# mandt-lab/shallow-ntc

Measured on AMD Instinct MI355X. Metric: decode Mpixels/s + (bpp, PSNR) on Kodak, two_layer_syn, higher is better.
Workload: dtype f32

## Files before the change

### shallow-ntc_amd/csrc/bf3_gemm.hip

```cpp
#include <algorithm>
#include <type_traits>
#include "sntc_internal.h"

namespace sntc {

typedef float f32x4 __attribute__((ext_vector_type(4)));
typedef float f32x16 __attribute__((ext_vector_type(16)));
typedef unsigned u32x4 __attribute__((ext_vector_type(4)));
typedef __bf16 bf16x8 __attribute__((ext_vector_type(8)));

namespace {

constexpr unsigned kOOR = 0x80000000u;
constexpr int kSpin = 1 << 22;

__device__ __forceinline__ float act_of(float v, int act) {
  switch (act) {
    case SNTC_ACT_RELU: return fmaxf(v, 0.0f);
    case SNTC_ACT_LEAKY_RELU: return v >= 0.0f ? v : 0.2f * v;
    case SNTC_ACT_SIGMOID: return 1.0f / (1.0f + expf(-v));
    default: return v;
  }
}

// ... 453 lines not shown
  using I1 = std::integral_constant<int, 1>;

  int mBc = 0, mBn = 0, mBn2 = 0;
  int mPc = 0, mP1 = 0, mP2 = 0;
  int nP = 0, nP_buf = 0, c_last = 0;
  int pm[NS - 1];
  auto start_piece = [&](const Piece& p, int rb) {
    init_loader(p, rb);
    const int n = __builtin_amdgcn_readfirstlane(p.k1 - p.k0);
    if (HALO) {
      issued = 0;
      const int c0 = ld_cc;
      c_last = __builtin_amdgcn_readfirstlane((p.k1 - 1) / g_T);
      rd_t = ld_t; rd_tx = ld_tx; rd_buf = 0;
      rd_shift = h_shift0 + ld_ty * (h_rowjump + (g_tw - 1) * h_coljump) + ld_tx * h_coljump;
      issue_patch(c0, 0);
      mPc = issued;
      if (h_nbufs == 3 && c0 + 1 <= c_last) issue_patch(c0 + 1, 1);
      mP1 = issued;
      mP2 = issued;
      nP = c0 + h_nbufs - 1;
      nP_buf = h_nbufs - 1;
#pragma unroll
      for (int q = 0; q < NS - 1; ++q) {
        if (q < n) issue(q);
        pm[q] = issued;
      }
      mBc = pm[0];
      mBn = pm[1];
    } else {
      if (n > 0) issue(0);
      if (n > 1) issue(1);
    }
  };

  int rb = 0;
  write_rinfo(P, rb);
  __syncthreads();
  start_piece(P, rb);
  while (true) {
    const int n = __builtin_amdgcn_readfirstlane(P.k1 - P.k0);
    if (P.consume >= 0) {
      if (tid == 0) {
        int spins = 0;
        while (__hip_atomic_load(a.sk_flags + P.consume, __ATOMIC_RELAXED, __HIP_MEMORY_SCOPE_AGENT) == 0) {
          __builtin_amdgcn_s_sleep(8);
          if (++spins > kSpin) {
            __hip_atomic_fetch_or(kargs().status, 1, __ATOMIC_RELAXED, __HIP_MEMORY_SCOPE_AGENT);
            break;
          }
        }
        __builtin_amdgcn_fence(__ATOMIC_ACQUIRE, "agent");
        asm volatile("s_waitcnt vmcnt(0)" ::: "memory");
      }
      __syncthreads();
      const __amdgpu_buffer_rsrc_t sr = __builtin_amdgcn_make_buffer_rsrc(
          a.sk_slab + (size_t)P.consume * (TM * TN * 16 * NT), 0, TM * TN * 16 * NT * 4, 0x00020000);
#pragma unroll
      for (int i = 0; i < TM; ++i)
#pragma unroll
        for (int j = 0; j < TN; ++j)
#pragma unroll
          for (int q = 0; q < 4; ++q) {
            const u32x4 v = __builtin_amdgcn_raw_buffer_load_b128(sr, tid * 16, ((i * TN + j) * 4 + q) * NT * 16, 0);
            const f32x4 f = __builtin_bit_cast(f32x4, v);
            acc[i][j][4 * q] = f[0]; acc[i][j][4 * q + 1] = f[1]; acc[i][j][4 * q + 2] = f[2]; acc[i][j][4 * q + 3] = f[3];
          }
    } else {
#pragma unroll
      for (int i = 0; i < TM; ++i)
#pragma unroll
        for (int j = 0; j < TN; ++j)
#pragma unroll
          for (int e = 0; e < 16; ++e) acc[i][j][e] = 0.0f;
    }

    Frag F;
    int s_cur = 0, s_n1 = 1, s_n2 = 2;
    if constexpr (HALO && DBUF) {
      Frag G;
      wait_vm(issued - max(mBc, mPc));
      __builtin_amdgcn_s_barrier();
      __builtin_amdgcn_sched_barrier(0);
      int mq[NS - 2];
#pragma unroll
      for (int q = 0; q < NS - 2; ++q) mq[q] = pm[q + 1];
      int s_rd = 0, s_is = NS - 1;
      auto mf = [&](const Frag& Fc, bool on, int q) {
        const int t = q / (TM * TN), i = (q / TN) % TM, j2 = q % TN;
        constexpr int PA[6] = {2, 0, 1, 1, 0, 0};
        constexpr int PB[6] = {0, 2, 1, 0, 1, 0};
        if (on && !SNTC_DBG(a, 64))
          acc[i][j2] = __builtin_amdgcn_mfma_f32_32x32x16_bf16(Fc.a[PA[t]][i], Fc.b[PB[t]][j2], acc[i][j2], 0, 0, 0);
        __builtin_amdgcn_sched_barrier(0);
      };
      auto step = [&](auto EDGE_, int j, Frag& Fc, Frag& Fn) {
        constexpr bool EDGE = decltype(EDGE_)::value;
        const bool mm = !EDGE || j >= 0, rd = (!EDGE || j + 1 < n) && (!SNTC_DBG(a, 8) || j < 1);
        static_assert(TM == 2 && TN == 2, "the slices below are laid out for a 64 x 64 wave tile (24 MFMAs per stage)");
        const char* src[TM];
        bool in[TM];
        const char* bsrc = ring + s_rd * SLOT + fb;
        int q = 0;
#pragma unroll
        for (int i = 0; i < TM; ++i) {
          const int prow = r_row[i] + rd_shift;
// ... 288 lines not shown
```

### shallow-ntc_amd/csrc/common.hip

```cpp
#include <algorithm>
#include <cstring>
#include "sntc_internal.h"

namespace sntc {

static thread_local std::string g_last_error;

void set_error(const std::string& msg) { g_last_error = msg; }

int fail(int code, const std::string& msg) {
  g_last_error = msg;
  return code;
}

int hip_fail(hipError_t e, const char* what) {
  g_last_error = std::string("HIP error in ") + what + ": " + hipGetErrorString(e);
  (void)hipGetLastError();
  return SNTC_ERR_HIP;
}

__global__ void __launch_bounds__(256) zero_words_kernel(uint32_t* __restrict__ p, size_t n) {
  for (size_t i = blockIdx.x * (size_t)blockDim.x + threadIdx.x; i < n; i += (size_t)gridDim.x * blockDim.x) p[i] = 0u;
}

int zero_async(void* p, size_t bytes, hipStream_t stream) {
  if (bytes == 0) return SNTC_OK;
  if ((bytes & 3u) || (reinterpret_cast<uintptr_t>(p) & 3u)) return fail(SNTC_ERR_BAD_SHAPE, "zero_async: unaligned range");
  const size_t n = bytes / 4;
  const int blocks = (int)std::min<size_t>((n + 255) / 256, 1024);
  hipLaunchKernelGGL(zero_words_kernel, dim3(blocks), dim3(256), 0, stream, reinterpret_cast<uint32_t*>(p), n);
  hipError_t e = hipGetLastError();
  if (e != hipSuccess) return hip_fail(e, "zero_async");
  return SNTC_OK;
}

}

extern "C" const char* sntc_last_error(void) { return sntc::g_last_error.c_str(); }

extern "C" int sntc_version(void) { return SNTC_VERSION; }

extern "C" int sntc_device_count(void) {
  int n = 0;
  if (hipGetDeviceCount(&n) != hipSuccess) {
    (void)hipGetLastError();
    return 0;
  }
  return n;
}

extern "C" int sntc_device_arch(int device, char* buf, size_t buflen) {
  if (!buf || buflen == 0) return sntc::fail(SNTC_ERR_BAD_SHAPE, "sntc_device_arch: null buffer");
  hipDeviceProp_t prop;
  if (sntc_device_count() <= device || device < 0) return sntc::fail(SNTC_ERR_NO_DEVICE, "no such HIP device");
  SNTC_HIP(hipGetDeviceProperties(&prop, device));
  std::strncpy(buf, prop.gcnArchName, buflen - 1);
  buf[buflen - 1] = 0;
  return SNTC_OK;
}
```

### shallow-ntc_amd/csrc/conv_plan.hip

```cpp
#include <algorithm>
#include <cstdio>
#include <cstdlib>
#include <array>
#include <atomic>
#include <map>
#include <mutex>
#include <cstdlib>
#include <vector>
#include "sntc_internal.h"

namespace sntc {

struct PackDesc {
  const float* w;
  float* wp;
  const int* taps;
  const unsigned* cols;
  int T, Cin, Cout, K, Ncol, kw, s, pt, pl, phase_mode, slab_major, out_major, bf3, rowpack;
};

__device__ __forceinline__ void pack_element(const PackDesc& d, size_t idx) {
  const int col = (int)(idx / d.K);
  const int k = (int)(idx - (size_t)col * d.K);
  float v = 0.0f;
// ... 102 lines not shown
  } g[kMaxGroups];
  float* bias = nullptr;
  int tile = 0;
  bool bf3 = false;
  bool rowpack = false;
  bool s3 = false;
  bool out_major = false;
  int dma = -1;
  bool no_stream_k = false;
  bool force_stream_k = false;
  int colm = -1;
  bool no_halo = false;
  float* w2f = nullptr;
  struct Choice { int variant = 0; int sk = 0; };
  mutable std::mutex tune_mu;
  std::map<std::array<int, 4>, Choice> tuned;
};
typedef sntc_conv_plan::Choice TuneChoice;

static const GGInstance* base_instance(const sntc_conv_plan* p, int v) {
  return p->s3 ? gg_find(v, kLoadVec, kStageDma, kFormPresplit) : gg_find(v, kLoadVec, kStageRing, kFormPlain);
}

extern "C" int sntc_conv_plan_set_tile(sntc_conv_plan* p, int variant) {
  if (!p) return fail(SNTC_ERR_BAD_SHAPE, "sntc_conv_plan_set_tile: null plan");
  if (variant != 0 && !base_instance(p, variant)) return fail(SNTC_ERR_UNSUPPORTED, "sntc_conv_plan_set_tile: unknown tile variant");
  p->tile = variant;
  return SNTC_OK;
}

static bool plan_dma(const sntc_conv_plan* p) {
  return p->dma > 0 && p->vec && p->d.prologue == SNTC_PRO_NONE && !p->bf3;
}

extern "C" int sntc_conv_plan_set_schedule(sntc_conv_plan* p, int flags) {
  if (!p) return fail(SNTC_ERR_BAD_SHAPE, "sntc_conv_plan_set_schedule: null plan");
  p->no_stream_k = (flags & 1) == 0;
  p->force_stream_k = (flags & 8) != 0;
  p->no_halo = (flags & 16) != 0;
  p->colm = (flags & 32) ? ((flags & 64) ? 1 : 0) : -1;
  p->dma = (flags & 4) ? ((flags & 2) ? 1 : 0) : -1;
  return SNTC_OK;
}

extern "C" void sntc_conv_plan_destroy(sntc_conv_plan* p) {
  if (!p) return;
  for (int i = 0; i < kMaxGroups; ++i) {
    if (p->g[i].wp) (void)hipFree(p->g[i].wp);
    if (p->g[i].taps) (void)hipFree(p->g[i].taps);
    if (p->g[i].cols) (void)hipFree(p->g[i].cols);
  }
  if (p->bias) (void)hipFree(p->bias);
  if (p->w2f) (void)hipFree(p->w2f);
  delete p;
}

static bool fusable_second(const sntc_conv_plan* p) {
  const sntc_conv_desc& b = p->d;
  return !p->up && !p->bf3 && b.kh == 1 && b.kw == 1 && b.stride == 1 && b.cin == 96 && b.cout == 192 &&
         b.prologue == SNTC_PRO_NONE && b.act == SNTC_ACT_NONE && p->ngroups == 1 && p->g[0].K == 96;
}

static int pack_fused_second(sntc_conv_plan* p, hipStream_t stream) {
  if (!fusable_second(p)) return SNTC_OK;
  if (!p->w2f) SNTC_HIP(hipMalloc(&p->w2f, sizeof(float) * 2 * 3 * 12 * 64 * 4));
  hipLaunchKernelGGL(pack_fused_w2_kernel, dim3(72), dim3(256), 0, stream, p->g[0].wp, p->w2f, p->g[0].K, p->g[0].Ncol);
  SNTC_HIP(hipGetLastError());
  return SNTC_OK;
}

static int build_plan(sntc_conv_plan* p, const float* weight, const float* bias, hipStream_t stream) {
  const sntc_conv_desc& d = p->d;
  const int k = d.kh, s = d.stride;
  struct HostGrp { std::vector<int> taps; std::vector<unsigned> cols; int q0y = 0, q0x = 0; bool uniform = true; };
  std::vector<HostGrp> groups;
  auto enc = [](int oyo, int oxo, int ch) { return ((unsigned)(oyo + 128) << 24) | ((unsigned)(oxo + 128) << 16) | (unsigned)ch; };

  if (!p->phase_mode) {
    HostGrp hg;
    for (int ky = 0; ky < d.kh; ++ky)
      for (int kx = 0; kx < (p->rowpack ? 1 : d.kw); ++kx) hg.taps.push_back((ky << 16) | kx);
    for (int ch = 0; ch < d.cout; ++ch) hg.cols.push_back(enc(0, 0, ch));
    groups.push_back(std::move(hg));
  } else {
    auto classes = [&](int kk, std::vector<std::pair<int, std::vector<int>>>& out) {
      for (int phi = 0; phi < s; ++phi) {
        const int cnt = (kk - phi + s - 1) / s;
        if (cnt <= 0) return false;
        bool found = false;
        for (auto& c : out)
          if (c.first == cnt) { c.second.push_back(phi); found = true; }
        if (!found) out.push_back({cnt, {phi}});
      }
      std::sort(out.begin(), out.end(), [](const auto& a, const auto& b) { return a.first > b.first; });
      return true;
    };
    std::vector<std::pair<int, std::vector<int>>> cy, cx;
    if (!classes(d.kh, cy) || !classes(d.kw, cx))
      return fail(SNTC_ERR_UNSUPPORTED, "transposed convolution with kernel < stride is not supported");
    for (auto& a : cy)
      for (auto& b : cx) {
        HostGrp hg;
        for (int jy = 0; jy < a.first; ++jy)
          for (int jx = 0; jx < b.first; ++jx) hg.taps.push_back((jy << 16) | jx);
        for (int py : a.second)
          for (int px : b.second)
// ... 511 lines not shown
  return conv_launch_info(p, n, h, w, 0, variant, nblocks, nullptr);
}

static int conv_forward_impl(const sntc_conv_plan* p, const sntc_conv_plan* p2, const float* x, int n, int h, int w, float* y,
                             const float* res, const float* aux, void* workspace, size_t workspace_bytes, void* stream,
                             const TuneChoice* force = nullptr, int ncols = 0) {
  if (!p || !x || !y) return fail(SNTC_ERR_BAD_SHAPE, "sntc_conv_forward: null argument");
  if (ncols != 0) {
    if (const char* why = columns_error(p, ncols)) return fail(SNTC_ERR_UNSUPPORTED, why);
    if (p2) return fail(SNTC_ERR_UNSUPPORTED, "column-limited launches: not the fused pair");
  }
  if (n < 1) return fail(SNTC_ERR_BAD_SHAPE, "sntc_conv_forward: empty batch");
  const sntc_conv_desc& d = p->d;
  const int epilogue = p2 ? p2->d.epilogue : d.epilogue;
  if (epilogue != SNTC_EPI_STORE && !res) return fail(SNTC_ERR_BAD_SHAPE, "epilogue needs `res`");
  if (epilogue == SNTC_EPI_GATE && !aux) return fail(SNTC_ERR_BAD_SHAPE, "gate epilogue needs `aux`");
  Geo g;
  int rc = geometry(p, h, w, &g);
  if (rc) return rc;
  const int64_t M = (int64_t)n * g.Qh * g.Qw;
  const int64_t x_bytes = (int64_t)n * h * w * d.cin * (p->s3 ? 6 : 4);
  if (M > 0x7fffffffLL || x_bytes >= (1LL << 31))
    return fail(SNTC_ERR_BAD_SHAPE, "sntc_conv_forward: input tensor must be < 2 GiB (32-bit buffer offsets); split the batch");
  if (p2 && M * p2->d.cout >= (1LL << 32)) return fail(SNTC_ERR_BAD_SHAPE, "sntc_conv_forward_fused: output too large; split the batch");
  const Sched sc = force ? schedule(p, g, n, false, force, ncols) : plan_schedule(p, g, n, h, w, p2 != nullptr, ncols);
  if (!sc.inst) return fail(SNTC_ERR_UNSUPPORTED, "sntc_conv_forward: no compiled instance for this plan and tile variant");
  const int64_t ws_floats = workspace_floats(p, M, sc, ncols);
  if (ws_floats > 0 && (!workspace || workspace_bytes < (size_t)ws_floats * 4))
    return fail(SNTC_ERR_BAD_SHAPE, "sntc_conv_forward: this call needs sntc_conv_workspace_bytes() of workspace "
                                    "(split-K slabs / stream-K hand-off)");
  const GGInstance& inst = *sc.inst;
  const Work wk = work_of(p, inst, M, ncols);
  if (sc.sk && wk.units != sc.units) return fail(SNTC_ERR_HIP, "sntc_conv_forward: schedule and launch disagree about the work units");
  GGArgs a{};
  a.ksplit = sc.ksplit;
  a.slab = static_cast<float*>(workspace);
  a.x = x; a.y = y; a.bias = p->bias; a.res = res; a.aux = aux;
  a.x_bytes = (unsigned)x_bytes;
  a.N = n; a.H = h; a.W = w; a.Cin = d.cin;
  a.Qh = g.Qh; a.Qw = g.Qw; a.M = (int)M;
  a.Ho = g.Ho; a.Wo = g.Wo; a.Cout = ncols > 0 ? ncols : d.cout;
  a.sA = g.sA; a.tstep = g.tstep; a.offy = g.offy; a.offx = g.offx; a.sO = g.sO;
  a.act = d.act; a.epi = epilogue; a.pro = d.prologue;
  a.ntm = wk.ntm;
  a.ngroups = p->ngroups;
  if (p2) { a.w2f = p2->w2f; a.bias2 = p2->bias; a.Cout2 = p2->d.cout; }
  a.status = gg_status_word();
  if (!a.status) return fail(SNTC_ERR_HIP, "sntc_conv_forward: the device tables of the current device are not initialised");
  a.sk = sc.sk ? 1 : 0;
  a.nworkers = sc.workers;
  a.units = wk.units;
  if (sc.sk) {
    a.sk_slab = static_cast<float*>(workspace);
    a.sk_flags = reinterpret_cast<int*>(a.sk_slab + (size_t)sc.workers * inst.slab_floats);
    a.slab = nullptr;
    if (int zrc = zero_async(a.sk_flags, sizeof(int) * sc.workers, (hipStream_t)stream)) return zrc;
  }
  int nb = 0;
  size_t slab_off = 0;
  for (int gi = 0; gi < p->ngroups; ++gi) {
    GGGroup& G = a.g[gi];
    G.wp = p->g[gi].wp; G.taps = p->g[gi].taps; G.cols = reinterpret_cast<const int*>(p->g[gi].cols);
    G.T = p->g[gi].T; G.K = p->g[gi].K; G.Ncol = launch_cols(p, gi, ncols); G.tw = p->g[gi].tw;
    G.ntn = wk.ntn[gi];
    G.steps = G.K / kStage;
    G.blk0 = nb;
    G.tile0 = wk.tile0[gi];
    G.unit0 = wk.unit0[gi];
    nb += G.ntn * a.ntm * sc.ksplit;
    G.slab_off = slab_off;
    G.q0y = p->g[gi].q0y; G.q0x = p->g[gi].q0x;
    slab_off += (size_t)sc.ksplit * M * G.Ncol;
  }
  a.tps = wk.tps;
  a.ups = (int)wk.ups;
  if (p->s3) a.order = p->dma == 0 ? 0 : 1;
  rc = gg_launch(inst, a, sc.sk ? sc.workers : nb, (hipStream_t)stream);
  if (rc || sc.sk || sc.ksplit <= 1) return rc;
  return gg_reduce_launch(a, (hipStream_t)stream);
}

extern "C" int sntc_conv_forward(const sntc_conv_plan* p, const float* x, int n, int h, int w, float* y,
                                 const float* res, const float* aux, void* workspace, size_t workspace_bytes,
                                 void* stream) {
  return conv_forward_impl(p, nullptr, x, n, h, w, y, res, aux, workspace, workspace_bytes, stream);
}

static void tune_candidates(const sntc_conv_plan* p, const Geo& g, int n, std::vector<std::pair<TuneChoice, Sched>>* out, int ncols = 0) {
  for (int v = 1; v <= kMaxVariant; ++v) {
    if (!base_instance(p, v)) continue;
    for (int sk = 1; sk >= 0; --sk) {
      TuneChoice c;
      c.variant = v;
      c.sk = sk;
      const Sched s = schedule(p, g, n, false, &c, ncols);
      if (!s.inst || s.inst->variant != v || (sk && !s.sk)) continue;
      out->push_back({c, s});
    }
  }
}

static int64_t conv_tune_workspace_bytes(const sntc_conv_plan* p, int n, int h, int w, int ncols) {
  if (!p) return 0;
  Geo g;
  if (geometry(p, h, w, &g)) return 0;
  std::vector<std::pair<TuneChoice, Sched>> cand;
  tune_candidates(p, g, n, &cand, ncols);
  int64_t m = 0;
  for (auto& c : cand) m = std::max(m, workspace_floats(p, (int64_t)n * g.Qh * g.Qw, c.second, ncols));
// ... 127 lines not shown

extern "C" int sntc_conv_columns_candidates(const sntc_conv_plan* p, int n, int h, int w, int ncols, int* variants, int* stream_k,
                                            int capacity) {
  if (columns_error(p, ncols)) { (void)fail(SNTC_ERR_UNSUPPORTED, columns_error(p, ncols)); return -1; }
  return conv_plan_candidates(p, n, h, w, ncols, variants, stream_k, capacity);
}

extern "C" int sntc_conv_columns_set_choice(sntc_conv_plan* p, int n, int h, int w, int ncols, int variant, int stream_k) {
  if (const char* why = columns_error(p, ncols)) return fail(SNTC_ERR_UNSUPPORTED, why);
  return conv_plan_set_choice(p, n, h, w, ncols, variant, stream_k);
}

extern "C" int sntc_conv_plan_drop_choice(sntc_conv_plan* p, int n, int h, int w, int ncols) {
  if (!p) return fail(SNTC_ERR_BAD_SHAPE, "sntc_conv_plan_drop_choice: null plan");
  std::lock_guard<std::mutex> lk(p->tune_mu);
  p->tuned.erase({n, h, w, ncols});
  return SNTC_OK;
}

extern "C" int sntc_conv_plan_clear_tuning(sntc_conv_plan* p) {
  if (!p) return fail(SNTC_ERR_BAD_SHAPE, "sntc_conv_plan_clear_tuning: null plan");
  std::lock_guard<std::mutex> lk(p->tune_mu);
  p->tuned.clear();
  return SNTC_OK;
}

static const char* fused_pair_error(const sntc_conv_plan* p, const sntc_conv_plan* p2) {
  if (!p || !p2) return "null plan";
  const sntc_conv_desc& a = p->d;
  if (p->up || p2->up || p->bf3 || p2->bf3) return "forward convolutions in fp32 only";
  if (!p->vec || a.cout != 96 || a.stride != 1 || a.prologue != SNTC_PRO_NONE || a.epilogue != SNTC_EPI_STORE || p->ngroups != 1)
    return "first plan: stride-1 convolution with Cin % 16 == 0 and 96 output channels, plain store";
  if (!fusable_second(p2) || !p2->w2f) return "second plan: 1x1 convolution 96 -> 192 without activation";
  return nullptr;
}

extern "C" int sntc_conv_fusable(const sntc_conv_plan* p, const sntc_conv_plan* p2) { return fused_pair_error(p, p2) ? 0 : 1; }

extern "C" int64_t sntc_conv_fused_workspace_bytes(const sntc_conv_plan* p, int n, int h, int w) {
  if (!p) return 0;
  Geo g;
  if (geometry(p, h, w, &g)) return 0;
  return 4 * workspace_floats(p, (int64_t)n * g.Qh * g.Qw, schedule(p, g, n, true));
}

extern "C" int sntc_conv_forward_fused(const sntc_conv_plan* p, const sntc_conv_plan* p2, const float* x, int n, int h, int w, float* y,
                                       const float* res, const float* aux, void* workspace, size_t workspace_bytes,
                                       void* stream) {
  if (const char* why = fused_pair_error(p, p2)) return fail(SNTC_ERR_UNSUPPORTED, why);
  return conv_forward_impl(p, p2, x, n, h, w, y, res, aux, workspace, workspace_bytes, stream);
}

extern "C" int sntc_conv_set_stream_k(int enabled) {
  g_stream_k_enabled.store(enabled ? 1 : 0, std::memory_order_relaxed);
  return SNTC_OK;
}

extern "C" int sntc_conv_get_stream_k(void) { return g_stream_k_enabled.load(std::memory_order_relaxed); }

__global__ void status_exchange_kernel(int* word, int* out) { *out = atomicExch(word, 0); }
__global__ void status_or_kernel(int* word, int flags) { atomicOr(word, flags); }

extern "C" int sntc_conv_status(int* flags, void* stream) {
  if (!flags) return fail(SNTC_ERR_BAD_SHAPE, "sntc_conv_status: null argument");
  int rc = gg_init();
  if (rc) return rc;
  int* word = gg_status_word();
  hipStream_t s = (hipStream_t)stream;
  hipLaunchKernelGGL(status_exchange_kernel, dim3(1), dim3(1), 0, s, word, word + 1);
  SNTC_HIP(hipGetLastError());
  SNTC_HIP(hipMemcpyAsync(flags, word + 1, sizeof(int), hipMemcpyDeviceToHost, s));
  SNTC_HIP(hipStreamSynchronize(s));
  return SNTC_OK;
}

extern "C" int sntc_conv_status_inject(int flags, void* stream) {
  int rc = gg_init();
  if (rc) return rc;
  hipLaunchKernelGGL(status_or_kernel, dim3(1), dim3(1), 0, (hipStream_t)stream, gg_status_word(), flags);
  SNTC_HIP(hipGetLastError());
  return SNTC_OK;
}
```

### shallow-ntc_amd/csrc/gather_gemm_kernel.h

```cpp
#pragma once
#include <algorithm>
#include <cstdlib>
#include <mutex>
#include <type_traits>
#include "sntc_internal.h"

namespace sntc {

typedef float f32x4 __attribute__((ext_vector_type(4)));
typedef float f32x16 __attribute__((ext_vector_type(16)));
typedef unsigned u32x4 __attribute__((ext_vector_type(4)));

constexpr unsigned kOutOfRange = 0x80000000u;
constexpr int kSpinLimit = 1 << 22;

__device__ __forceinline__ float apply_act(float v, int act) {
  switch (act) {
    case SNTC_ACT_RELU: return fmaxf(v, 0.0f);
    case SNTC_ACT_LEAKY_RELU: return v >= 0.0f ? v : 0.2f * v;
    case SNTC_ACT_SIGMOID: return 1.0f / (1.0f + expf(-v));
    default: return v;
  }
}

// ... 525 lines not shown
  f32x16 acc[TM][TN];
  auto mfma3 = [&](const Frag3& F) {
    constexpr int PA[6] = {2, 0, 1, 1, 0, 0};
    constexpr int PB[6] = {0, 2, 1, 0, 1, 0};
#pragma unroll
    for (int t = 0; t < (BF3 ? 6 : 0); ++t)
#pragma unroll
      for (int i = 0; i < TM; ++i)
#pragma unroll
        for (int j = 0; j < TN; ++j)
          acc[i][j] = __builtin_amdgcn_mfma_f32_32x32x16_bf16(F.a[BF3 ? PA[t] : 0][i], F.b[BF3 ? PB[t] : 0][j], acc[i][j], 0, 0, 0);
  };
  auto mfma_group = [&](const Frag& F) {
    if (SNTC_DBG(a, 64)) return;
#pragma unroll
    for (int e = 0; e < 4; ++e)
#pragma unroll
      for (int i = 0; i < TM; ++i)
#pragma unroll
        for (int j = 0; j < TN; ++j)
          acc[i][j] = FUSE2 ? __builtin_amdgcn_mfma_f32_32x32x2f32(F.b[j][e], F.a[i][e], acc[i][j], 0, 0, 0)
                            : __builtin_amdgcn_mfma_f32_32x32x2f32(F.a[i][e], F.b[j][e], acc[i][j], 0, 0, 0);
  };

  int rb = 0;
  Regs R0, R1;
  write_rinfo(P, rb);
  __syncthreads();
  init_loader(P, rb);
  int dma_issued = 0;
  if (DMA) {
    const int n = P.k1 - P.k0;
    for (; dma_issued < RING - 1 && dma_issued < n; ++dma_issued) dma_stage(dma_issued);
  } else {
    const int n = P.k1 - P.k0;
    if (n > 0) load_regs(R0);
    if (RBUF && n > 1) load_regs(R1);
  }

  while (true) {
    const int n = P.k1 - P.k0;
    if (P.consume >= 0) {
      if (tid == 0) {
        int spins = 0;
        while (__hip_atomic_load(a.sk_flags + P.consume, __ATOMIC_RELAXED, __HIP_MEMORY_SCOPE_AGENT) == 0) {
          __builtin_amdgcn_s_sleep(8);
          if (++spins > kSpinLimit) {
            __hip_atomic_fetch_or(fresh_args().status, 1, __ATOMIC_RELAXED, __HIP_MEMORY_SCOPE_AGENT);
            break;
          }
        }
        __builtin_amdgcn_fence(__ATOMIC_ACQUIRE, "agent");
        asm volatile("s_waitcnt vmcnt(0)" ::: "memory");
      }
      __syncthreads();
      const __amdgpu_buffer_rsrc_t sr = __builtin_amdgcn_make_buffer_rsrc(
          a.sk_slab + (size_t)P.consume * (TM * TN * 16 * 256), 0, TM * TN * 16 * 256 * 4, 0x00020000);
#pragma unroll
      for (int i = 0; i < TM; ++i)
#pragma unroll
        for (int j = 0; j < TN; ++j)
#pragma unroll
          for (int q = 0; q < 4; ++q) {
            const f32x4 v = buf_load(sr, (unsigned)tid * 16u, (unsigned)((i * TN + j) * 4 + q) * 4096u);
            acc[i][j][4 * q] = v[0]; acc[i][j][4 * q + 1] = v[1]; acc[i][j][4 * q + 2] = v[2]; acc[i][j][4 * q + 3] = v[3];
          }
    } else {
#pragma unroll
      for (int i = 0; i < TM; ++i)
#pragma unroll
        for (int j = 0; j < TN; ++j)
#pragma unroll
          for (int e = 0; e < 16; ++e) acc[i][j][e] = 0.0f;
    }

    Frag F0, F1;
    if (DMA) {
      for (; dma_issued < RING - 1 && dma_issued < n; ++dma_issued) dma_stage(dma_issued);
      using Yes = std::integral_constant<bool, true>;
      using No = std::integral_constant<bool, false>;
      auto wait_first = [&](auto I) {
        constexpr int i = decltype(I)::value;
        if constexpr (i > 2) {
          if (n >= i) { dma_wait(std::integral_constant<int, i - 2>{}); return true; }
        }
        return false;
      };
      if (!first_of_desc<RING - 1, 3>(wait_first)) dma_wait(std::integral_constant<int, 0>{});
      __builtin_amdgcn_s_barrier();
      __builtin_amdgcn_sched_barrier(0);
      if (n > 0) read_frag(F0, 0, 0);
      auto dstep = [&](int j, auto LD, auto PF, auto REM) {
        if (decltype(LD)::value) dma_stage((j + RING - 1) & (RING - 1));
        read_frag(F1, j & (RING - 1), 1);
        mfma_group(F0);
        if (decltype(PF)::value) read_frag(F0, (j + 1) & (RING - 1), 0);
        mfma_group(F1);
        if (decltype(LD)::value) {
          constexpr int NW = A_CH + B_CH, NR = TM + TN, NM = 4 * TM * TN;
          __builtin_amdgcn_sched_group_barrier(0x008, 1, 0);
          __builtin_amdgcn_sched_group_barrier(0x020, NW, 0);
          __builtin_amdgcn_sched_group_barrier(0x008, 1, 0);
          __builtin_amdgcn_sched_group_barrier(0x100, NR, 0);
          __builtin_amdgcn_sched_group_barrier(0x008, NM - 2, 0);
          __builtin_amdgcn_sched_group_barrier(0x008, 1, 0);
          __builtin_amdgcn_sched_group_barrier(0x100, NR, 0);
// ... 283 lines not shown
```

### shallow-ntc_amd/csrc/sntc_internal.h

```cpp
#pragma once
#include <hip/hip_runtime.h>
#include <stdint.h>
#include <string>
#include "../../include/sntc.h"

namespace sntc {

void set_error(const std::string& msg);
int fail(int code, const std::string& msg);
int hip_fail(hipError_t e, const char* what);
int zero_async(void* p, size_t bytes, hipStream_t stream);

#define SNTC_HIP(expr)                                         \
  do {                                                         \
    hipError_t _e = (expr);                                    \
    if (_e != hipSuccess) return ::sntc::hip_fail(_e, #expr);  \
  } while (0)

constexpr int kMaxGroups = 4;

#ifdef SNTC_DIAG
#define SNTC_DBG(a, bit) (((a).dbg & (bit)) != 0)
#else
#define SNTC_DBG(a, bit) false
#endif

struct GGGroup {
  const float* wp;
  const int* taps;
  const int* cols;
  int T;
  int tw;
  int K;
  int Ncol;
  int ntn;
  int blk0;
  size_t slab_off;
  int q0y, q0x;
  int steps;
  int tile0;
  long long unit0;
};

struct GGArgs {
  const float* x;
  float* y;
  const float* bias;
  const float* res;
  const float* aux;
  unsigned x_bytes;
  int N, H, W, Cin;
  int Qh, Qw, M;
  int Ho, Wo, Cout;
  int sA, tstep, offy, offx, sO;
  int act, epi, pro;
  int ntm;
  int ksplit;
  float* slab;
  int sk;
  int nworkers;
  long long units;
  int tps, ups;
  float* sk_slab;
  int* sk_flags;
// ... 60 lines not shown
```

### shallow-ntc_amd/csrc/syn_fused.hip

```cpp
#include <algorithm>
#include <cmath>
#include <cstdio>
#include <cstdlib>
#include <cstring>
#include <mutex>
#include <vector>
#include "sntc_internal.h"

#include "rb_common.h"

namespace sntc {
namespace syn {

using rb::buf_load;
using rb::buf_store;
using rb::kOOB;

constexpr int kNT = 3;
constexpr int kRows = 32 * kNT;
constexpr int kUnit = kRows * 16;
constexpr int kRing = 8;
constexpr int kLead = 5;
constexpr int kPSlots = 3;
constexpr int kPPMax = 512;
// ... 440 lines not shown
        for (int c = 0; c < CP; ++c) {
          const int vi = sl * CP + c;
          tv[c] = acc[vi >> 4][vi & 15] + bias[c];
        }
        float o[CH];
        if (act == 1 || act == 2) {
          float av[CH];
#pragma unroll
          for (int ic = 0; ic < CH; ++ic) av[ic] = fabsf(tv[ic]);
          f32x2 nrm[CH / 2];
#pragma unroll
          for (int jp = 0; jp < CH / 2; ++jp) nrm[jp] = *reinterpret_cast<const f32x2*>(beta + 2 * jp);
#pragma unroll
          for (int ic = 0; ic < CH; ++ic)
#pragma unroll
            for (int jp = 0; jp < CH / 2; ++jp) {
              const f32x2 g = *reinterpret_cast<const f32x2*>(gamma + ic * CH + 2 * jp);
              const f32x2 pr = g * av[ic];
              nrm[jp] = nrm[jp] + pr;
            }
          if (act == 1) {
#pragma unroll
            for (int jc = 0; jc < CH; ++jc) o[jc] = tv[jc] * nrm[jc >> 1][jc & 1];
          } else {
#pragma unroll
            for (int jc = 0; jc < CH; ++jc) o[jc] = tv[jc] / nrm[jc >> 1][jc & 1];
          }
        } else if (act == 3) {
#pragma unroll
          for (int jc = 0; jc < CH; ++jc) o[jc] = fmaxf(tv[jc], 0.0f);
        } else if (act == 4) {
#pragma unroll
          for (int jc = 0; jc < CH; ++jc) o[jc] = tv[jc] >= 0.0f ? tv[jc] : 0.2f * tv[jc];
        } else {
#pragma unroll
          for (int jc = 0; jc < CH; ++jc) o[jc] = tv[jc];
        }
        if (RES) {
#pragma unroll
          for (int jc = 0; jc < CH; ++jc) o[jc] = o[jc] + tv[CH + jc];
        }
        const unsigned ph0 = up->ph[sl], ph1 = up->ph[SPH + sl];
        const unsigned ph = h ? ph1 : ph0;
        const int ry = (int)(ph >> 8), rx = (int)(ph & 255u);
        const bool ok = pvalid && ph != 0xffffffffu;
        const unsigned off = ok ? (unsigned)(((qy * a.s + ry) * Wo + qx * a.s + rx) * (CH * 4)) : kOOB;
#pragma unroll
        for (int c4 = 0; c4 < CH; c4 += 4) buf_store(vs, f32x4{o[c4], o[c4 + 1], o[c4 + 2], o[c4 + 3]}, off, c4 * 4);
      }
    }
    if (!more) break;
  }
  asm volatile("s_waitcnt vmcnt(0)" ::: "memory");
}

__global__ void __launch_bounds__(256) syn_pack_kernel(const float* __restrict__ w, const SynUnit* __restrict__ units, int nunits,
                                                        SynGeom G, int nslab, int total_steps, float* __restrict__ wpack) {
  const size_t total = (size_t)total_steps * kUnit;
  for (size_t idx = blockIdx.x * (size_t)blockDim.x + threadIdx.x; idx < total; idx += (size_t)gridDim.x * blockDim.x) {
    const int gstep = (int)(idx / kUnit);
    const int rem = (int)(idx - (size_t)gstep * kUnit);
    const int R = rem >> 4, pos = rem & 15;
    const int k16 = (((pos >> 2) ^ ((R >> 2) & 3)) << 2) + (pos & 3);
    int u = 0;
    for (int i = 1; i < nunits; ++i)
      if (gstep >= units[i].step0) u = i;
    const SynUnit U = units[u];
    const int local = gstep - U.step0;
    const int cc = local / U.ns, j = local - cc * U.ns;
    wpack[idx] = pack_value(G, U, cc, j, R, k16, w);
  }
}

__global__ void syn_tables_kernel(const float* b1, const float* beta, const float* gamma, int cp, int ch, float* out) {
  const int i = blockIdx.x * blockDim.x + threadIdx.x;
  if (i < cp) out[i] = b1 ? b1[i] : 0.0f;
  else if (i < cp + ch) out[i] = beta ? beta[i - cp] : 1.0f;
  else if (i < cp + ch + ch * ch) out[i] = gamma ? gamma[i - cp - ch] : 0.0f;
}

struct HostPlan {
  SynGeom G{};
  int ch = 0, has_res = 0;
  std::vector<SynUnit> units;
  int total_steps = 0;
  int nslab = 0;
};

static bool dim_ok(int k, int s, int pt) {
  for (int r = 0; r < s; ++r) {
    const int phi = (r + pt) % s, qo = (r + pt) / s, cnt = (k - phi + s - 1) / s;
    if (cnt < 1 || qo > 1 || qo - cnt + 1 < -1) return false;
  }
  return true;
}

static unsigned phase_mask(const SynGeom& G, int ry, int rx) {
  unsigned m = 0;
  for (int si = 0; si < 9; ++si) {
    const int dy = 1 - si / 3, dx = 1 - si % 3;
    const int phy = (ry + G.pt) % G.s, qoy = (ry + G.pt) / G.s, cy = (G.k - phy + G.s - 1) / G.s;
    const int phx = (rx + G.pt) % G.s, qox = (rx + G.pt) / G.s, cx = (G.k - phx + G.s - 1) / G.s;
    const int jy = qoy - dy, jx = qox - dx;
    if (jy >= 0 && jy < cy && jx >= 0 && jx < cx) m |= 1u << si;
  }
  return m;
// ... 101 lines not shown
  int rc = SNTC_OK;
  int num_cus = 0;
};
SynDevice g_syndev[kMaxDev];

template <int CP, bool RES>
static int set_attr() {
  SNTC_HIP(hipFuncSetAttribute(reinterpret_cast<const void*>(&syn_kernel<CP, RES>), hipFuncAttributeMaxDynamicSharedMemorySize,
                               (int)SynCfg<CP, RES>::LDS));
  return SNTC_OK;
}

static int syn_init(int* num_cus) {
  int dev = 0;
  SNTC_HIP(hipGetDevice(&dev));
  if (dev < 0 || dev >= kMaxDev) return fail(SNTC_ERR_UNSUPPORTED, "device index beyond the synthesis tables");
  SynDevice& D = g_syndev[dev];
  std::call_once(D.once, [&] {
    D.rc = [&]() -> int {
      hipDeviceProp_t prop;
      SNTC_HIP(hipGetDeviceProperties(&prop, dev));
      D.num_cus = prop.multiProcessorCount;
      if (int rc = set_attr<12, false>()) return rc;
      if (int rc = set_attr<24, false>()) return rc;
      if (int rc = set_attr<24, true>()) return rc;
      if (int rc = set_attr<48, false>()) return rc;
      if (int rc = set_attr<48, true>()) return rc;
      return SNTC_OK;
    }();
  });
  *num_cus = D.num_cus;
  return D.rc;
}

}
}

using namespace sntc;
using namespace sntc::syn;

struct sntc_syn_plan {
  HostPlan P;
  int act_kind = 0;
  float* wpack = nullptr;
  SynUnit* units = nullptr;
  float* tables = nullptr;
  int max_workgroups = 0;
};

static void syn_free(sntc_syn_plan* p) {
  if (p->wpack) (void)hipFree(p->wpack);
  if (p->units) (void)hipFree(p->units);
  if (p->tables) (void)hipFree(p->tables);
  delete p;
}

static int syn_pack(sntc_syn_plan* p, const float* w1, const float* b1, const float* beta, const float* gamma, hipStream_t s) {
  const HostPlan& P = p->P;
  const size_t total = (size_t)P.total_steps * kUnit;
  const int blocks = (int)std::min<size_t>((total + 255) / 256, 4096);
  hipLaunchKernelGGL(syn_pack_kernel, dim3(blocks), dim3(256), 0, s, w1, p->units, (int)P.units.size(), P.G, P.nslab, P.total_steps, p->wpack);
  const int nt = P.G.cp + P.ch + P.ch * P.ch;
  hipLaunchKernelGGL(syn_tables_kernel, dim3((nt + 255) / 256), dim3(256), 0, s, b1, beta, gamma, P.G.cp, P.ch, p->tables);
  hipError_t e = hipGetLastError();
  if (e != hipSuccess) return hip_fail(e, "synthesis weight packing");
  return SNTC_OK;
}

extern "C" int sntc_syn_supported(int k, int stride, int cin, int ch, int has_res) {
  HostPlan P;
  if (k < 1 || stride < 1 || ch < 1) return 0;
  return build_host_plan(k, stride, cin, ch, has_res ? 1 : 0, &P) == SNTC_OK ? 1 : 0;
}

extern "C" int sntc_syn_plan_create(int k, int stride, int cin, int ch, int has_res, int act_kind, const float* w1, const float* b1,
                                    const float* beta, const float* gamma, void* stream, sntc_syn_plan** plan) {
  if (!plan || !w1) return fail(SNTC_ERR_BAD_SHAPE, "sntc_syn_plan_create: null argument");
  if (act_kind < 0 || act_kind > 4) return fail(SNTC_ERR_UNSUPPORTED, "sntc_syn_plan_create: unknown activation");
  if ((act_kind == 1 || act_kind == 2) && (!beta || !gamma)) return fail(SNTC_ERR_BAD_SHAPE, "sntc_syn_plan_create: GDN parameters missing");
  if (k < 1 || stride < 1 || ch < 1) return fail(SNTC_ERR_BAD_SHAPE, "sntc_syn_plan_create: bad sizes");
  auto* p = new sntc_syn_plan();
  if (int rc = build_host_plan(k, stride, cin, ch, has_res ? 1 : 0, &p->P)) { delete p; return rc; }
  int cus = 0;
  if (int rc = syn_init(&cus)) { delete p; return rc; }
  p->act_kind = act_kind;
  const HostPlan& P = p->P;
  const int nt = P.G.cp + P.ch + P.ch * P.ch;
  if (hipMalloc(&p->wpack, sizeof(float) * (size_t)P.total_steps * kUnit) != hipSuccess ||
      hipMalloc(&p->units, sizeof(SynUnit) * P.units.size()) != hipSuccess || hipMalloc(&p->tables, sizeof(float) * nt) != hipSuccess) {
    syn_free(p);
    return fail(SNTC_ERR_HIP, "sntc_syn_plan_create: out of device memory");
  }
  hipStream_t s = (hipStream_t)stream;
  if (hipMemcpyAsync(p->units, P.units.data(), sizeof(SynUnit) * P.units.size(), hipMemcpyHostToDevice, s) != hipSuccess ||
      hipStreamSynchronize(s) != hipSuccess) {
    syn_free(p);
    return fail(SNTC_ERR_HIP, "sntc_syn_plan_create: unit table upload");
  }
  if (int rc = syn_pack(p, w1, b1, beta, gamma, s)) { syn_free(p); return rc; }
  *plan = p;
  return SNTC_OK;
}

extern "C" int sntc_syn_plan_update(sntc_syn_plan* p, const float* w1, const float* b1, const float* beta, const float* gamma, void* stream) {
  if (!p || !w1) return fail(SNTC_ERR_BAD_SHAPE, "sntc_syn_plan_update: null argument");
  if ((p->act_kind == 1 || p->act_kind == 2) && (!beta || !gamma)) return fail(SNTC_ERR_BAD_SHAPE, "sntc_syn_plan_update: GDN parameters missing");
  return syn_pack(p, w1, b1, beta, gamma, (hipStream_t)stream);
}

extern "C" void sntc_syn_plan_destroy(sntc_syn_plan* p) {
  if (p) syn_free(p);
}

extern "C" int sntc_syn_plan_set_workgroups(sntc_syn_plan* p, int max_workgroups) {
  if (!p || max_workgroups < 0) return fail(SNTC_ERR_BAD_SHAPE, "sntc_syn_plan_set_workgroups: bad argument");
  p->max_workgroups = max_workgroups;
  return SNTC_OK;
}

extern "C" int64_t sntc_syn_flops(const sntc_syn_plan* p, int64_t latent_pixels) {
  if (!p || latent_pixels < 0) return -1;
  return 2 * latent_pixels * p->P.G.k * p->P.G.k * p->P.G.cin * p->P.G.cp;
}

extern "C" int64_t sntc_syn_workspace_bytes(const sntc_syn_plan* p) { return p ? 256 : -1; }

extern "C" int sntc_syn_forward(const sntc_syn_plan* p, const sntc_syn_batch* batches, int nbatches, void* workspace, size_t workspace_bytes,
                                void* stream) {
  if (!p || !batches || !workspace) return fail(SNTC_ERR_BAD_SHAPE, "sntc_syn_forward: null argument");
  if (nbatches < 1 || nbatches > kMaxSynGroups) return fail(SNTC_ERR_BAD_SHAPE, "sntc_syn_forward: 1 .. 4 batches per call");
  if (workspace_bytes < 256) return fail(SNTC_ERR_BAD_SHAPE, "sntc_syn_forward: workspace smaller than sntc_syn_workspace_bytes()");
  const HostPlan& P = p->P;
  SynArgs a{};
  int64_t tiles = 0;
  int ng = 0;
  for (int i = 0; i < nbatches; ++i) {
    const sntc_syn_batch& b = batches[i];
    if (b.n < 0 || b.h < 0 || b.w < 0) return fail(SNTC_ERR_BAD_SHAPE, "sntc_syn_forward: negative size");
    if (b.n == 0 || b.h == 0 || b.w == 0) continue;
    if (!b.y_hat || !b.hidden) return fail(SNTC_ERR_BAD_SHAPE, "sntc_syn_forward: null tensor");
    if (kTileM + 2 * b.w + 2 > kPPMax) return fail(SNTC_ERR_UNSUPPORTED, "sntc_syn_forward: latent rows wider than 127 pixels");
    const int64_t hw = (int64_t)b.h * b.w;
    if (hw * P.G.cin * 4 >= (1LL << 31) || hw * P.G.s * P.G.s * P.ch * 4 >= (1LL << 31))
      return fail(SNTC_ERR_BAD_SHAPE, "sntc_syn_forward: one image's tensor of 2 GiB or more");
    SynGroup& g = a.g[ng++];
    g.x = b.y_hat; g.v = b.hidden; g.n = b.n; g.h = b.h; g.w = b.w;
    g.tile0 = (int)tiles;
    g.tpi = (int)((hw + kTileM - 1) / kTileM);
    tiles += (int64_t)b.n * g.tpi;
    if (tiles * (int64_t)P.units.size() >= (1LL << 30)) return fail(SNTC_ERR_BAD_SHAPE, "sntc_syn_forward: too many work items");
  }
  if (ng == 0) return SNTC_OK;
  int cus = 0;
  if (int rc = syn_init(&cus)) return rc;
  a.wpack = p->wpack; a.units = p->units; a.tables = p->tables;
  a.queue = reinterpret_cast<int*>(workspace);
  a.wbytes = (unsigned)((size_t)P.total_steps * kUnit * 4);
  a.nunits = (int)P.units.size(); a.ntiles = (int)tiles; a.nitems = a.nunits * a.ntiles;
  a.cin = P.G.cin; a.nslab = P.nslab; a.s = P.G.s; a.act_kind = p->act_kind;
  a.ngroups = ng;
#ifdef SNTC_DIAG
  if (const char* e = getenv("SNTC_SYN_DBG")) a.dbg = atoi(e);
#endif
  hipStream_t s = (hipStream_t)stream;
  if (int zrc = zero_async(workspace, 64, s)) return zrc;
  const int grid = std::min<int64_t>(a.nitems, p->max_workgroups > 0 ? p->max_workgroups : cus);
  const void* fn = nullptr;
  size_t lds = 0;
  const int cp = P.G.cp;
  if (cp == 12 && !P.has_res) { fn = reinterpret_cast<const void*>(&syn_kernel<12, false>); lds = SynCfg<12, false>::LDS; }
  else if (cp == 24 && !P.has_res) { fn = reinterpret_cast<const void*>(&syn_kernel<24, false>); lds = SynCfg<24, false>::LDS; }
  else if (cp == 24 && P.has_res) { fn = reinterpret_cast<const void*>(&syn_kernel<24, true>); lds = SynCfg<24, true>::LDS; }
  else if (cp == 48 && !P.has_res) { fn = reinterpret_cast<const void*>(&syn_kernel<48, false>); lds = SynCfg<48, false>::LDS; }
  else if (cp == 48 && P.has_res) { fn = reinterpret_cast<const void*>(&syn_kernel<48, true>); lds = SynCfg<48, true>::LDS; }
  else return fail(SNTC_ERR_UNSUPPORTED, "sntc_syn_forward: no kernel for this width");
  void* params[] = {&a};
  hipError_t e = hipLaunchKernel(fn, dim3(grid), dim3(512), params, lds, s);
  if (e != hipSuccess) return hip_fail(e, "synthesis launch");
  return SNTC_OK;
}

extern "C" int sntc_syn_selfcheck(int k, int stride, int cin, int ch, int has_res, int h, int w, unsigned seed, double* max_err) {
  if (!max_err) return fail(SNTC_ERR_BAD_SHAPE, "sntc_syn_selfcheck: null argument");
  HostPlan P;
  if (int rc = build_host_plan(k, stride, cin, ch, has_res ? 1 : 0, &P)) return rc;
  if (h < 1 || w < 1 || kTileM + 2 * w + 2 > kPPMax) return fail(SNTC_ERR_BAD_SHAPE, "sntc_syn_selfcheck: bad image size");
  const SynGeom G = P.G;
  const int cp = G.cp, s = G.s;
  unsigned st = seed * 2654435761u + 12345u;
  auto rnd = [&]() { st = st * 1664525u + 1013904223u; return (double)((st >> 8) & 0xffff) / 32768.0 - 1.0; };
  std::vector<float> wk((size_t)k * k * cp * cin), x((size_t)h * w * cin);
  for (auto& v : wk) v = (float)rnd();
  for (auto& v : x) v = (float)rnd();
  const int Ho = h * s, Wo = w * s;
  std::vector<double> ref((size_t)Ho * Wo * cp, 0.0), got((size_t)Ho * Wo * cp, 0.0);
  std::vector<int> hits((size_t)Ho * Wo, 0);
  for (int iy = 0; iy < h; ++iy)
    for (int ix = 0; ix < w; ++ix)
      for (int ky = 0; ky < k; ++ky)
        for (int kx = 0; kx < k; ++kx) {
          const int oy = iy * s + ky - G.pt, ox = ix * s + kx - G.pt;
          if (oy < 0 || oy >= Ho || ox < 0 || ox >= Wo) continue;
          for (int c = 0; c < cp; ++c) {
            double acc = 0.0;
            for (int ci = 0; ci < cin; ++ci) acc += (double)x[((size_t)iy * w + ix) * cin + ci] * wk[((size_t)(ky * k + kx) * cp + c) * cin + ci];
            ref[((size_t)oy * Wo + ox) * cp + c] += acc;
          }
        }
  const int sph = 48 / cp;
  const int HW = h * w;
  for (const SynUnit& U : P.units)
    for (int m = 0; m < HW; ++m) {
      const int qy = m / w, qx = m % w;
      double acc[kRows];
      for (int R = 0; R < kRows; ++R) acc[R] = 0.0;
      for (int cc = 0; cc < P.nslab; ++cc)
        for (int j = 0; j < U.ns; ++j) {
          const int si = unit_shift(U, j), dy = 1 - si / 3, dx = 1 - si % 3;
// ... 58 lines not shown
```

Measured before the change: 3994.

## Self-reset work-queue and stream-K flags in-kernel instead of zeroing per launch

Replaces the per-launch zeroing kernels for the synthesis work queue and the stream-K flags with persistent device buffers that the kernels reset themselves. The last workgroup clears the queue counter, and each consumer clears its flag after reading it. This removes one small kernel launch before each synthesis and conv call. The cost is a host-side map and mutex, re-zeroing after timeouts or toggles, and the risk of stale state if a launch aborts or two streams share a buffer concurrently.

Result: no change. 3989 (-0.1%).

```diff
diff --git a/shallow-ntc_amd/csrc/bf3_gemm.hip b/shallow-ntc_amd/csrc/bf3_gemm.hip
--- a/shallow-ntc_amd/csrc/bf3_gemm.hip
+++ b/shallow-ntc_amd/csrc/bf3_gemm.hip
@@ -529,6 +529,7 @@
         }
         __builtin_amdgcn_fence(__ATOMIC_ACQUIRE, "agent");
         asm volatile("s_waitcnt vmcnt(0)" ::: "memory");
+        __hip_atomic_store(a.sk_flags + P.consume, 0, __ATOMIC_RELAXED, __HIP_MEMORY_SCOPE_AGENT);
       }
       __syncthreads();
       const __amdgpu_buffer_rsrc_t sr = __builtin_amdgcn_make_buffer_rsrc(
diff --git a/shallow-ntc_amd/csrc/common.hip b/shallow-ntc_amd/csrc/common.hip
--- a/shallow-ntc_amd/csrc/common.hip
+++ b/shallow-ntc_amd/csrc/common.hip
@@ -1,5 +1,8 @@
 #include <algorithm>
 #include <cstring>
+#include <map>
+#include <mutex>
+#include <tuple>
 #include "sntc_internal.h"
 
 namespace sntc {
@@ -34,6 +37,97 @@
   return SNTC_OK;
 }
 
+namespace {
+struct RearmKey {
+  const void* owner;
+  hipStream_t stream;
+  int64_t k0, k1;
+  size_t words;
+  bool operator<(const RearmKey& o) const {
+    return std::tie(owner, stream, k0, k1, words) < std::tie(o.owner, o.stream, o.k0, o.k1, o.words);
+  }
+};
+struct RearmBlock { int* p; size_t words; int device; };
+std::mutex g_rearm_mu;
+std::map<RearmKey, RearmBlock> g_rearm;
+std::multimap<const void*, RearmBlock> g_rearm_captured;
+constexpr int kRearmDevices = 16;
+hipStream_t g_rearm_stream[kRearmDevices] = {};
+
+struct RelaxedCapture {
+  hipStreamCaptureMode mode = hipStreamCaptureModeRelaxed;
+  RelaxedCapture() { (void)hipThreadExchangeStreamCaptureMode(&mode); }
+  ~RelaxedCapture() { (void)hipThreadExchangeStreamCaptureMode(&mode); }
+};
+
+int rearm_zero(const RearmBlock& b) {
+  if (b.device < 0 || b.device >= kRearmDevices) return fail(SNTC_ERR_UNSUPPORTED, "device index beyond the re-arm streams");
+  hipStream_t& s = g_rearm_stream[b.device];
+  if (!s) SNTC_HIP(hipStreamCreateWithFlags(&s, hipStreamNonBlocking));
+  SNTC_HIP(hipMemsetAsync(b.p, 0, b.words * sizeof(int), s));
+  SNTC_HIP(hipStreamSynchronize(s));
+  return SNTC_OK;
+}
+}
+
+int* rearm_words(const void* owner, hipStream_t stream, int64_t key0, int64_t key1, size_t words) {
+  if (words == 0) { (void)fail(SNTC_ERR_BAD_SHAPE, "rearm_words: empty block"); return nullptr; }
+  hipStreamCaptureStatus cs = hipStreamCaptureStatusNone;
+  if (stream && hipStreamIsCapturing(stream, &cs) != hipSuccess) { (void)hipGetLastError(); cs = hipStreamCaptureStatusNone; }
+  const bool capturing = cs == hipStreamCaptureStatusActive;
+  const RearmKey key{owner, stream, key0, key1, words};
+  std::lock_guard<std::mutex> lk(g_rearm_mu);
+  if (!capturing) {
+    auto it = g_rearm.find(key);
+    if (it != g_rearm.end()) return it->second.p;
+  }
+  RelaxedCapture relaxed;
+  RearmBlock b{nullptr, words, 0};
+  if (hipGetDevice(&b.device) != hipSuccess || hipMalloc(&b.p, words * sizeof(int)) != hipSuccess) {
+    (void)hipGetLastError();
+    (void)fail(SNTC_ERR_HIP, "rearm_words: out of device memory");
+    return nullptr;
+  }
+  if (rearm_zero(b)) { (void)hipFree(b.p); return nullptr; }
+  if (capturing) g_rearm_captured.insert({owner, b});
+  else g_rearm[key] = b;
+  return b.p;
+}
+
+void rearm_release(const void* owner) {
+  std::lock_guard<std::mutex> lk(g_rearm_mu);
+  for (auto it = g_rearm.begin(); it != g_rearm.end();) {
+    if (it->first.owner == owner) { (void)hipFree(it->second.p); it = g_rearm.erase(it); }
+    else ++it;
+  }
+  auto range = g_rearm_captured.equal_range(owner);
+  for (auto it = range.first; it != range.second; ++it) (void)hipFree(it->second.p);
+  g_rearm_captured.erase(range.first, range.second);
+}
+
+int rearm_zero_all() {
+  std::lock_guard<std::mutex> lk(g_rearm_mu);
+  if (g_rearm.empty() && g_rearm_captured.empty()) return SNTC_OK;
+  int dev = 0;
+  SNTC_HIP(hipGetDevice(&dev));
+  for (int d = 0; d < kRearmDevices; ++d) {
+    bool used = false;
+    for (auto& kv : g_rearm) used |= kv.second.device == d;
+    for (auto& kv : g_rearm_captured) used |= kv.second.device == d;
+    if (!used) continue;
+    SNTC_HIP(hipSetDevice(d));
+    SNTC_HIP(hipDeviceSynchronize());
+    for (auto& kv : g_rearm)
+      if (kv.second.device == d)
+        if (int rc = rearm_zero(kv.second)) { (void)hipSetDevice(dev); return rc; }
+    for (auto& kv : g_rearm_captured)
+      if (kv.second.device == d)
+        if (int rc = rearm_zero(kv.second)) { (void)hipSetDevice(dev); return rc; }
+  }
+  SNTC_HIP(hipSetDevice(dev));
+  return SNTC_OK;
+}
+
 }
 
 extern "C" const char* sntc_last_error(void) { return sntc::g_last_error.c_str(); }
diff --git a/shallow-ntc_amd/csrc/conv_plan.hip b/shallow-ntc_amd/csrc/conv_plan.hip
--- a/shallow-ntc_amd/csrc/conv_plan.hip
+++ b/shallow-ntc_amd/csrc/conv_plan.hip
@@ -178,6 +178,7 @@
   }
   if (p->bias) (void)hipFree(p->bias);
   if (p->w2f) (void)hipFree(p->w2f);
+  rearm_release(p);
   delete p;
 }
 
@@ -795,9 +796,9 @@
   a.units = wk.units;
   if (sc.sk) {
     a.sk_slab = static_cast<float*>(workspace);
-    a.sk_flags = reinterpret_cast<int*>(a.sk_slab + (size_t)sc.workers * inst.slab_floats);
     a.slab = nullptr;
-    if (int zrc = zero_async(a.sk_flags, sizeof(int) * sc.workers, (hipStream_t)stream)) return zrc;
+    a.sk_flags = rearm_words(p, (hipStream_t)stream, ((int64_t)n << 32) | (unsigned)ncols, ((int64_t)h << 32) | (unsigned)w, (size_t)sc.workers);
+    if (!a.sk_flags) return SNTC_ERR_HIP;
   }
   int nb = 0;
   size_t slab_off = 0;
@@ -1031,7 +1032,8 @@
 }
 
 extern "C" int sntc_conv_set_stream_k(int enabled) {
-  g_stream_k_enabled.store(enabled ? 1 : 0, std::memory_order_relaxed);
+  const int was = g_stream_k_enabled.exchange(enabled ? 1 : 0, std::memory_order_relaxed);
+  if (enabled && !was) return rearm_zero_all();
   return SNTC_OK;
 }
 
@@ -1050,6 +1052,7 @@
   SNTC_HIP(hipGetLastError());
   SNTC_HIP(hipMemcpyAsync(flags, word + 1, sizeof(int), hipMemcpyDeviceToHost, s));
   SNTC_HIP(hipStreamSynchronize(s));
+  if (*flags & 1) return rearm_zero_all();
   return SNTC_OK;
 }
 
diff --git a/shallow-ntc_amd/csrc/gather_gemm_kernel.h b/shallow-ntc_amd/csrc/gather_gemm_kernel.h
--- a/shallow-ntc_amd/csrc/gather_gemm_kernel.h
+++ b/shallow-ntc_amd/csrc/gather_gemm_kernel.h
@@ -601,6 +601,7 @@
         }
         __builtin_amdgcn_fence(__ATOMIC_ACQUIRE, "agent");
         asm volatile("s_waitcnt vmcnt(0)" ::: "memory");
+        __hip_atomic_store(a.sk_flags + P.consume, 0, __ATOMIC_RELAXED, __HIP_MEMORY_SCOPE_AGENT);
       }
       __syncthreads();
       const __amdgpu_buffer_rsrc_t sr = __builtin_amdgcn_make_buffer_rsrc(
diff --git a/shallow-ntc_amd/csrc/sntc_internal.h b/shallow-ntc_amd/csrc/sntc_internal.h
--- a/shallow-ntc_amd/csrc/sntc_internal.h
+++ b/shallow-ntc_amd/csrc/sntc_internal.h
@@ -10,6 +10,10 @@
 int fail(int code, const std::string& msg);
 int hip_fail(hipError_t e, const char* what);
 int zero_async(void* p, size_t bytes, hipStream_t stream);
+
+int* rearm_words(const void* owner, hipStream_t stream, int64_t key0, int64_t key1, size_t words);
+void rearm_release(const void* owner);
+int rearm_zero_all();
 
 #define SNTC_HIP(expr)                                         \
   do {                                                         \
diff --git a/shallow-ntc_amd/csrc/syn_fused.hip b/shallow-ntc_amd/csrc/syn_fused.hip
--- a/shallow-ntc_amd/csrc/syn_fused.hip
+++ b/shallow-ntc_amd/csrc/syn_fused.hip
@@ -516,6 +516,15 @@
     if (!more) break;
   }
   asm volatile("s_waitcnt vmcnt(0)" ::: "memory");
+  if (tid == 0) {
+    int* q = syn_args().queue;
+    __builtin_amdgcn_fence(__ATOMIC_RELEASE, "agent");
+    asm volatile("s_waitcnt vmcnt(0)" ::: "memory");
+    if (atomicInc(reinterpret_cast<unsigned*>(q + 1), gridDim.x - 1) == gridDim.x - 1) {
+      __builtin_amdgcn_fence(__ATOMIC_ACQUIRE, "agent");
+      __hip_atomic_store(q, 0, __ATOMIC_RELAXED, __HIP_MEMORY_SCOPE_AGENT);
+    }
+  }
 }
 
 __global__ void __launch_bounds__(256) syn_pack_kernel(const float* __restrict__ w, const SynUnit* __restrict__ units, int nunits,
@@ -723,6 +732,7 @@
   if (p->wpack) (void)hipFree(p->wpack);
   if (p->units) (void)hipFree(p->units);
   if (p->tables) (void)hipFree(p->tables);
+  rearm_release(p);
   delete p;
 }
 
@@ -825,7 +835,9 @@
   int cus = 0;
   if (int rc = syn_init(&cus)) return rc;
   a.wpack = p->wpack; a.units = p->units; a.tables = p->tables;
-  a.queue = reinterpret_cast<int*>(workspace);
+  hipStream_t s = (hipStream_t)stream;
+  a.queue = rearm_words(p, s, 0, 0, 16);
+  if (!a.queue) return SNTC_ERR_HIP;
   a.wbytes = (unsigned)((size_t)P.total_steps * kUnit * 4);
   a.nunits = (int)P.units.size(); a.ntiles = (int)tiles; a.nitems = a.nunits * a.ntiles;
   a.cin = P.G.cin; a.nslab = P.nslab; a.s = P.G.s; a.act_kind = p->act_kind;
@@ -833,8 +845,6 @@
 #ifdef SNTC_DIAG
   if (const char* e = getenv("SNTC_SYN_DBG")) a.dbg = atoi(e);
 #endif
-  hipStream_t s = (hipStream_t)stream;
-  if (int zrc = zero_async(workspace, 64, s)) return zrc;
   const int grid = std::min<int64_t>(a.nitems, p->max_workgroups > 0 ? p->max_workgroups : cus);
   const void* fn = nullptr;
   size_t lds = 0;
```
